# DrSleep/nas-segm-pytorch

Hardware: AMD Instinct MI355X
Metric: images/sec (fwd+bwd+optimizer step) WACV arch0 2048x1024 bs=4/GPU (higher is better)
Workload: dtype f32

## Files before the change

### nas-segm-pytorch_amd/csrc/irdw.hip

```cpp
#include "dw_common.h"

namespace {

#ifndef NASSEG_IR_BWD_MINB
#define NASSEG_IR_BWD_MINB 1
#endif
#ifndef NASSEG_IR_FWD_MINB
#define NASSEG_IR_FWD_MINB 1
#endif
constexpr int kIrMaxTiles = 12;
constexpr int kIrMaxWaves = 4;

__device__ __forceinline__ f32x4 mfma16(float a, float b, f32x4 c) {
  return __builtin_amdgcn_mfma_f32_16x16x4f32(a, b, c, 0, 0, 0);
}

template <int CTRL>
__device__ __forceinline__ float dpp_shift0(float v) {
  return __int_as_float(__builtin_amdgcn_update_dpp(0, __float_as_int(v), CTRL, 0xF, 0xF, true));
}
__device__ __forceinline__ float4 from_left(float4 v) {
  return make_float4(dpp_shift0<0x111>(v.x), dpp_shift0<0x111>(v.y), dpp_shift0<0x111>(v.z), dpp_shift0<0x111>(v.w));
}
__device__ __forceinline__ float4 from_right(float4 v) {
  return make_float4(dpp_shift0<0x101>(v.x), dpp_shift0<0x101>(v.y), dpp_shift0<0x101>(v.z), dpp_shift0<0x101>(v.w));
}
__device__ __forceinline__ float4 round_like_storage(float4 v) {
#ifdef NASSEG_BF16
  v = make_float4(bf16_to_f32(f32_to_bf16(v.x)), bf16_to_f32(f32_to_bf16(v.y)), bf16_to_f32(f32_to_bf16(v.z)),
                  bf16_to_f32(f32_to_bf16(v.w)));
#endif
  return v;
}

struct IrCommon {
  const act_t* x;
  const float* w1;
  const float* in_scale;
  const float* in_shift;
  int in_act;
  const float* sc1;
  const float* sh1;
  int act1;
  int B, H, W, K, C, Ho, Wo;
  int strips, chunks, rows_per_chunk, items;
};

template <int KT, bool PRO>
struct IrLane {
  float aw[KT][4];
  int koff[KT];
  float4 psc[KT], psh[KT];
  float plo, phi;
};
template <int KT, bool PRO>
__device__ __forceinline__ IrLane<KT, PRO> ir_lane(const IrCommon& q, int t, int j, int kg) {
  IrLane<KT, PRO> l;
#pragma unroll
  for (int kb = 0; kb < KT; ++kb) {
    const int k0 = 16 * kb + 4 * kg;
    const bool kok = k0 < q.K;
    l.koff[kb] = kok ? k0 : 0;
#pragma unroll
    for (int c = 0; c < 4; ++c) l.aw[kb][c] = kok ? q.w1[(size_t)(16 * t + j) * q.K + k0 + c] : 0.f;
    if (PRO) {
      l.psc[kb] = (q.in_scale && kok) ? ld4(q.in_scale + k0) : make_float4(1.f, 1.f, 1.f, 1.f);
      l.psh[kb] = (q.in_shift && kok) ? ld4(q.in_shift + k0) : f4zero();
    }
  }
  l.plo = q.in_act ? 0.f : -INFINITY;
  l.phi = q.in_act == NASSEG_ACT_RELU6 ? 6.f : INFINITY;
  return l;
}
template <int KT, bool PRO>
struct IrRawX {
  float4 v[KT];
};
template <int KT, bool PRO>
__device__ __forceinline__ IrRawX<KT, PRO> ir_load(const IrLane<KT, PRO>& l, const act_t* xp) {
  IrRawX<KT, PRO> r;
#pragma unroll
  for (int kb = 0; kb < KT; ++kb) r.v[kb] = lda4(xp + l.koff[kb]);
  return r;
}
template <int KT, bool PRO>
__device__ __forceinline__ float4 ir_mma(const IrLane<KT, PRO>& l, const IrRawX<KT, PRO>& r) {
  f32x4 acc = (f32x4){0.f, 0.f, 0.f, 0.f};
#pragma unroll
  for (int kb = 0; kb < KT; ++kb) {
    float4 v = r.v[kb];
    if (PRO) {
      v = fma4(v, l.psc[kb], l.psh[kb]);
      v.x = __builtin_amdgcn_fmed3f(v.x, l.plo, l.phi);
      v.y = __builtin_amdgcn_fmed3f(v.y, l.plo, l.phi);
      v.z = __builtin_amdgcn_fmed3f(v.z, l.plo, l.phi);
      v.w = __builtin_amdgcn_fmed3f(v.w, l.plo, l.phi);
    }
    acc = mfma16(l.aw[kb][0], v.x, acc);
    acc = mfma16(l.aw[kb][1], v.y, acc);
    acc = mfma16(l.aw[kb][2], v.z, acc);
    acc = mfma16(l.aw[kb][3], v.w, acc);
  }
  return round_like_storage(make_float4(acc[0], acc[1], acc[2], acc[3]));
}

struct IrFwdArgs {
  IrCommon c;
  const float* wdw;
  act_t* z2;
  float* stats;
};

template <int STRIDE, int KT, bool PRO>
__global__ __launch_bounds__(64 * kIrMaxWaves, NASSEG_IR_FWD_MINB) void irdw_fwd_kernel(IrFwdArgs a) {
  const IrCommon& q = a.c;
  const int lane = threadIdx.x & 63, t = blockIdx.y * (blockDim.x >> 6) + (threadIdx.x >> 6);
  const int j = lane & 15, kg = lane >> 4;
  const int C = q.C, K = q.K, H = q.H, W = q.W, Ho = q.Ho, Wo = q.Wo;
  const int c4 = 4 * t + kg;
  const IrLane<KT, PRO> ln = ir_lane<KT, PRO>(q, t, j, kg);
  const float4 sc1 = ld4(q.sc1 + 4 * c4), sh1 = ld4(q.sh1 + 4 * c4);
  const float lo1 = q.act1 ? 0.f : -INFINITY, hi1 = q.act1 == NASSEG_ACT_RELU6 ? 6.f : INFINITY;
  float4 wd[9];
#pragma unroll
  for (int tp = 0; tp < 9; ++tp) wd[tp] = ld4(a.wdw + (size_t)tp * C + 4 * c4);
  double dsum[4] = {0.0, 0.0, 0.0, 0.0}, dsq[4] = {0.0, 0.0, 0.0, 0.0};
  const bool out_lane = STRIDE == 1 ? (j >= 1 && j <= 14) : ((j & 1) && j <= 13);

  for (int item = blockIdx.x; item < q.items; item += gridDim.x) {
    const int s = item % q.strips;
    const int rest = item / q.strips;
    const int ch = rest % q.chunks, b = rest / q.chunks;
    const int oy0 = ch * q.rows_per_chunk;
    const int oy1 = oy0 + q.rows_per_chunk < Ho ? oy0 + q.rows_per_chunk : Ho;
    const int col = 14 * s - 1 + j;
    const bool colok = col >= 0 && col < W;
    const int colc = col < 0 ? 0 : (col >= W ? W - 1 : col);
    const int ox = STRIDE == 1 ? col : 7 * s + (j >> 1);
    const bool outok = out_lane && ox < Wo;
    const act_t* xb = q.x + ((size_t)b * H * W + colc) * K;
    act_t* zb = a.z2 + ((size_t)b * Ho * Wo + (outok ? ox : 0)) * C + 4 * c4;
    float4 fs = f4zero(), fq = f4zero();
    auto fetch = [&](int iy) {
      return ir_load<KT, PRO>(ln, xb + (size_t)(iy < 0 ? 0 : (iy >= H ? H - 1 : iy)) * W * K);
    };
    auto make_row = [&](const IrRawX<KT, PRO>& raw, int iy, float4& L, float4& M, float4& R) {
      const float4 z = ir_mma<KT, PRO>(ln, raw);
      float4 a1 = fma4(z, sc1, sh1);
      a1.x = __builtin_amdgcn_fmed3f(a1.x, lo1, hi1);
      a1.y = __builtin_amdgcn_fmed3f(a1.y, lo1, hi1);
      a1.z = __builtin_amdgcn_fmed3f(a1.z, lo1, hi1);
      a1.w = __builtin_amdgcn_fmed3f(a1.w, lo1, hi1);
      a1 = keep_if(a1, colok && iy >= 0 && iy < H);
      M = a1;
      L = from_left(a1);
      R = from_right(a1);
    };
    auto emit = [&](int oy, const float4& A0, const float4& A1, const float4& A2, const float4& B0, const float4& B1,
                    const float4& B2, const float4& C0, const float4& C1, const float4& C2) {
      float4 o = mul4(wd[0], A0);
      o = fma4(wd[1], A1, o);
      o = fma4(wd[2], A2, o);
      o = fma4(wd[3], B0, o);
      o = fma4(wd[4], B1, o);
      o = fma4(wd[5], B2, o);
      o = fma4(wd[6], C0, o);
      o = fma4(wd[7], C1, o);
      o = fma4(wd[8], C2, o);
      if (outok) sta4(zb + (size_t)oy * Wo * C, o);
      const float4 m = keep_if(o, outok);
      fs = add4(fs, m);
      fq = fma4(m, m, fq);
    };
    float4 L0, M0, R0, L1, M1, R1, L2, M2, R2;
    if (STRIDE == 1) {
      IrRawX<KT, PRO> ra = fetch(oy0 - 1), rb = fetch(oy0);
      make_row(ra, oy0 - 1, L0, M0, R0);
      ra = fetch(oy0 + 1);
      make_row(rb, oy0, L1, M1, R1);
      int oy = oy0;
      for (; oy + 2 < oy1; oy += 3) {
        rb = fetch(oy + 2);
        make_row(ra, oy + 1, L2, M2, R2);
        emit(oy, L0, M0, R0, L1, M1, R1, L2, M2, R2);
        ra = fetch(oy + 3);
        make_row(rb, oy + 2, L0, M0, R0);
        emit(oy + 1, L1, M1, R1, L2, M2, R2, L0, M0, R0);
        rb = fetch(oy + 4);
        make_row(ra, oy + 3, L1, M1, R1);
        emit(oy + 2, L2, M2, R2, L0, M0, R0, L1, M1, R1);
        ra = rb;
      }
      if (oy < oy1) {
        rb = fetch(oy + 2);
        make_row(ra, oy + 1, L2, M2, R2);
        emit(oy, L0, M0, R0, L1, M1, R1, L2, M2, R2);
        if (oy + 1 < oy1) {
          make_row(rb, oy + 2, L0, M0, R0);
          emit(oy + 1, L1, M1, R1, L2, M2, R2, L0, M0, R0);
        }
      }
    } else {
      IrRawX<KT, PRO> ra = fetch(2 * oy0 - 1), rb = fetch(2 * oy0);
      make_row(ra, 2 * oy0 - 1, L0, M0, R0);
      ra = fetch(2 * oy0 + 1);
      int oy = oy0;
      for (; oy + 1 < oy1; oy += 2) {
        make_row(rb, 2 * oy, L1, M1, R1);
        rb = fetch(2 * oy + 2);
        make_row(ra, 2 * oy + 1, L2, M2, R2);
        ra = fetch(2 * oy + 3);
        emit(oy, L0, M0, R0, L1, M1, R1, L2, M2, R2);
        make_row(rb, 2 * oy + 2, L1, M1, R1);
        rb = fetch(2 * oy + 4);
        make_row(ra, 2 * oy + 3, L0, M0, R0);
        ra = fetch(2 * oy + 5);
        emit(oy + 1, L2, M2, R2, L1, M1, R1, L0, M0, R0);
      }
      if (oy < oy1) {
        make_row(rb, 2 * oy, L1, M1, R1);
        make_row(ra, 2 * oy + 1, L2, M2, R2);
        emit(oy, L0, M0, R0, L1, M1, R1, L2, M2, R2);
      }
    }
    dsum[0] += (double)fs.x; dsum[1] += (double)fs.y; dsum[2] += (double)fs.z; dsum[3] += (double)fs.w;
    dsq[0] += (double)fq.x; dsq[1] += (double)fq.y; dsq[2] += (double)fq.z; dsq[3] += (double)fq.w;
  }
#pragma unroll
  for (int r = 0; r < 4; ++r) {
    dsum[r] = row16_allsum(dsum[r]);
    dsq[r] = row16_allsum(dsq[r]);
  }
  if (j == 0) {
    float* row = a.stats + (size_t)blockIdx.x * 2 * C + 4 * c4;
    *reinterpret_cast<float4*>(row) = make_float4((float)dsum[0], (float)dsum[1], (float)dsum[2], (float)dsum[3]);
    *reinterpret_cast<float4*>(row + C) = make_float4((float)dsq[0], (float)dsq[1], (float)dsq[2], (float)dsq[3]);
  }
}

struct IrBwdArgs {
  IrCommon c;
  const float* mu1;
  const float* is1;
  const act_t* g;
  const act_t* z2;
  const float* wdw;
  int flip;
  act_t* ge;
  float* partial;
  float* stats;
  const float* sc2; const float* sh2; const float* mu2; const float* is2; const float* sums2;
  int train2, act2;
  float invM;
};

struct IrDz {
  float4 ca, cb, cd, cs;
};
__device__ __forceinline__ IrDz ir_dz_const(const IrBwdArgs& a, int c4) {
  IrDz k;
  const int C = a.c.C;
  k.ca = ld4(a.sc2 + c4 * 4);
  k.cs = a.act2 ? ld4(a.sh2 + c4 * 4) : f4zero();
  k.cb = f4zero();
  k.cd = f4zero();
  if (a.train2) {
    const float4 is = ld4(a.is2 + c4 * 4), mu = ld4(a.mu2 + c4 * 4);
    const float4 s0 = ld4(a.sums2 + c4 * 4), s1 = ld4(a.sums2 + C + c4 * 4);
    const float m = a.invM;
    k.cb = make_float4(-k.ca.x * is.x * (s1.x * m), -k.ca.y * is.y * (s1.y * m), -k.ca.z * is.z * (s1.z * m),
                       -k.ca.w * is.w * (s1.w * m));
    k.cd = make_float4(k.ca.x * (mu.x * is.x * (s1.x * m) - s0.x * m), k.ca.y * (mu.y * is.y * (s1.y * m) - s0.y * m),
                       k.ca.z * (mu.z * is.z * (s1.z * m) - s0.z * m), k.ca.w * (mu.w * is.w * (s1.w * m) - s0.w * m));
  }
  return k;
}
struct IrRaw {
  float4 g, z;
  bool ok;
};
__device__ __forceinline__ IrRaw ir_dz_load(const IrBwdArgs& a, int b, int oy, int ox, int c4) {
  IrRaw r;
  const int Ho = a.c.Ho, Wo = a.c.Wo;
  r.ok = oy >= 0 && oy < Ho && ox >= 0 && ox < Wo;
  const int oyc = oy < 0 ? 0 : (oy >= Ho ? Ho - 1 : oy), oxc = ox < 0 ? 0 : (ox >= Wo ? Wo - 1 : ox);
  const size_t off = (((size_t)b * Ho + oyc) * Wo + oxc) * a.c.C + c4 * 4;
  r.g = lda4(a.g + off);
  r.z = lda4(a.z2 + off);
  return r;
}
__device__ __forceinline__ float4 ir_dz_make(const ActSel& act2, const IrDz& k, const IrRaw& r) {
  const float4 y = fma4(r.z, k.ca, k.cs);
  const float4 gv = make_float4(r.g.x * act_mask(y.x, act2), r.g.y * act_mask(y.y, act2), r.g.z * act_mask(y.z, act2),
                                r.g.w * act_mask(y.w, act2));
  return keep_if(round_like_storage(fma4(gv, k.ca, fma4(r.z, k.cb, k.cd))), r.ok);
}

template <int STRIDE, int KT, bool PRO>
__global__ __launch_bounds__(64 * kIrMaxWaves, NASSEG_IR_BWD_MINB) void irdw_bwd_kernel(IrBwdArgs a) {
  const IrCommon& q = a.c;
  const int lane = threadIdx.x & 63, t = blockIdx.y * (blockDim.x >> 6) + (threadIdx.x >> 6);
  const int j = lane & 15, kg = lane >> 4;
  const int C = q.C, K = q.K, H = q.H, W = q.W;
  const int c4 = 4 * t + kg;
  const IrLane<KT, PRO> ln = ir_lane<KT, PRO>(q, t, j, kg);
  const float4 sc1 = ld4(q.sc1 + 4 * c4), sh1 = ld4(q.sh1 + 4 * c4);
  const float4 mu1 = ld4(a.mu1 + 4 * c4), is1 = ld4(a.is1 + 4 * c4);
  const float lo1 = q.act1 ? 0.f : -INFINITY, hi1 = q.act1 == NASSEG_ACT_RELU6 ? 6.f : INFINITY;
  const IrDz kc = ir_dz_const(a, c4);
  const ActSel sel1 = act_sel(q.act1), sel2 = act_sel(a.act2);
  float4 lw[9];
#pragma unroll
  for (int tp = 0; tp < 9; ++tp) lw[tp] = ld4(a.wdw + (size_t)(a.flip ? 8 - tp : tp) * C + 4 * c4);
  float4 dwa[9];
#pragma unroll
  for (int tp = 0; tp < 9; ++tp) dwa[tp] = f4zero();
  float4 ssum[2] = {f4zero(), f4zero()};
  auto finish = [&](float4& o, float4 z1, bool ok) {
    const float4 y = fma4(z1, sc1, sh1);
    o.x *= act_mask(y.x, sel1);
    o.y *= act_mask(y.y, sel1);
    o.z *= act_mask(y.z, sel1);
    o.w *= act_mask(y.w, sel1);
    const float4 v = keep_if(o, ok);
    const float4 xh = make_float4((z1.x - mu1.x) * is1.x, (z1.y - mu1.y) * is1.y, (z1.z - mu1.z) * is1.z,
                                  (z1.w - mu1.w) * is1.w);
    ssum[0] = add4(ssum[0], v);
    ssum[1] = fma4(v, xh, ssum[1]);
  };
  auto activated = [&](float4 z1) {
    float4 v = fma4(z1, sc1, sh1);
    v.x = __builtin_amdgcn_fmed3f(v.x, lo1, hi1);
    v.y = __builtin_amdgcn_fmed3f(v.y, lo1, hi1);
    v.z = __builtin_amdgcn_fmed3f(v.z, lo1, hi1);
    v.w = __builtin_amdgcn_fmed3f(v.w, lo1, hi1);
    return v;
  };

  for (int item = blockIdx.x; item < q.items; item += gridDim.x) {
    const int s = item % q.strips;
    const int rest = item / q.strips;
    const int ch = rest % q.chunks, b = rest / q.chunks;
    const int r0 = ch * q.rows_per_chunk;
    if (STRIDE == 1) {
      const int r1 = r0 + q.rows_per_chunk < H ? r0 + q.rows_per_chunk : H;
      const int ix = 14 * s - 1 + j;
      const bool live = j >= 1 && j <= 14 && ix < W;
      const int xc = ix < 0 ? 0 : (ix >= W ? W - 1 : ix);
      const bool colok = ix >= 0 && ix < W;
      const act_t* xcol = q.x + ((size_t)b * H * W + xc) * K;
      float4 dl[3], dm[3], dr[3];
      auto make_dz = [&](const IrRaw& raw, float4& L, float4& M, float4& R) {
        IrRaw r = raw;
        r.ok = r.ok && colok;
        M = ir_dz_make(sel2, kc, r);
        L = from_left(M);
        R = from_right(M);
      };
      make_dz(ir_dz_load(a, b, r0 - 1, xc, c4), dl[1], dm[1], dr[1]);
      make_dz(ir_dz_load(a, b, r0, xc, c4), dl[2], dm[2], dr[2]);
      IrRaw nxt = ir_dz_load(a, b, r0 + 1, xc, c4), nxt2 = ir_dz_load(a, b, r0 + 2, xc, c4);
      IrRawX<KT, PRO> xnxt = ir_load<KT, PRO>(ln, xcol + (size_t)r0 * W * K);
      IrRawX<KT, PRO> xnxt2 = ir_load<KT, PRO>(ln, xcol + (size_t)(r0 + 1 < H ? r0 + 1 : H - 1) * W * K);
      for (int iy = r0; iy < r1; ++iy) {
        const IrRaw cur = nxt;
        const IrRawX<KT, PRO> xcur = xnxt;
        nxt = nxt2;
        xnxt = xnxt2;
        nxt2 = ir_dz_load(a, b, iy + 3, xc, c4);
        xnxt2 = ir_load<KT, PRO>(ln, xcol + (size_t)(iy + 2 < H ? iy + 2 : H - 1) * W * K);
        const float4 z1 = ir_mma<KT, PRO>(ln, xcur);
        dl[0] = dl[1]; dm[0] = dm[1]; dr[0] = dr[1];
        dl[1] = dl[2]; dm[1] = dm[2]; dr[1] = dr[2];
        make_dz(cur, dl[2], dm[2], dr[2]);
        const float4 xa = keep_if(activated(z1), live);
        float4 o = f4zero();
#pragma unroll
        for (int ty = 0; ty < 3; ++ty) {
          o = fma4(lw[ty * 3 + 0], dr[2 - ty], o);
          dwa[ty * 3 + 0] = fma4(xa, dr[2 - ty], dwa[ty * 3 + 0]);
          o = fma4(lw[ty * 3 + 1], dm[2 - ty], o);
          dwa[ty * 3 + 1] = fma4(xa, dm[2 - ty], dwa[ty * 3 + 1]);
          o = fma4(lw[ty * 3 + 2], dl[2 - ty], o);
          dwa[ty * 3 + 2] = fma4(xa, dl[2 - ty], dwa[ty * 3 + 2]);
        }
        finish(o, z1, live);
        if (live) sta4(a.ge + (((size_t)b * H + iy) * W + ix) * C + c4 * 4, o);
      }
    } else {
      const int Hq = (H + 1) >> 1, Wq = (W + 1) >> 1;
      const int r1 = r0 + q.rows_per_chunk < Hq ? r0 + q.rows_per_chunk : Hq;
      const int xq = 15 * s + j;
      const bool live = j <= 14 && xq < Wq;
      const int xqc = xq < Wq ? xq : Wq - 1;
      float4 d[2][2];
      auto make_dz = [&](const IrRaw& raw, float4& M, float4& R) {
        M = ir_dz_make(sel2, kc, raw);
        R = from_right(M);
      };
      auto fetch_quad = [&](int aq, IrRawX<KT, PRO> (&dst)[2][2]) {
#pragma unroll
        for (int py = 0; py < 2; ++py)
#pragma unroll
          for (int px = 0; px < 2; ++px) {
            const int iy = 2 * aq + py, ix = 2 * xqc + px;
            dst[py][px] = ir_load<KT, PRO>(ln, q.x + (((size_t)b * H + (iy < H ? iy : H - 1)) * W + (ix < W ? ix : W - 1)) * K);
          }
      };
      make_dz(ir_dz_load(a, b, r0, xq, c4), d[1][0], d[1][1]);
      IrRaw nxt = ir_dz_load(a, b, r0 + 1, xq, c4);
      IrRawX<KT, PRO> xnxt[2][2];
      fetch_quad(r0, xnxt);
      for (int aq = r0; aq < r1; ++aq) {
        const IrRaw cur = nxt;
        IrRawX<KT, PRO> xcur[2][2];
#pragma unroll
        for (int py = 0; py < 2; ++py)
#pragma unroll
          for (int px = 0; px < 2; ++px) xcur[py][px] = xnxt[py][px];
        nxt = ir_dz_load(a, b, aq + 2, xq, c4);
        fetch_quad(aq + 1 < Hq ? aq + 1 : aq, xnxt);
        d[0][0] = d[1][0];
        d[0][1] = d[1][1];
        make_dz(cur, d[1][0], d[1][1]);
#pragma unroll
        for (int py = 0; py < 2; ++py)
#pragma unroll
          for (int px = 0; px < 2; ++px) {
            const int iy = 2 * aq + py, ix = 2 * xqc + px;
            const bool ok = live && iy < H && ix < W;
            const float4 z1 = ir_mma<KT, PRO>(ln, xcur[py][px]);
            const float4 xa = keep_if(activated(z1), ok);
            float4 o = f4zero();
#pragma unroll
            for (int ty = 0; ty < 3; ++ty)
#pragma unroll
              for (int tx = 0; tx < 3; ++tx) {
                if (((ty + 1) & 1) != py || ((tx + 1) & 1) != px) continue;
                const int ry = (py + 1 - ty) / 2, rx = (px + 1 - tx) / 2;
                const float4 dv = d[ry][rx];
                o = fma4(lw[ty * 3 + tx], dv, o);
                dwa[ty * 3 + tx] = fma4(xa, dv, dwa[ty * 3 + tx]);
              }
            finish(o, z1, ok);
            if (ok) sta4(a.ge + (((size_t)b * H + iy) * W + 2 * xq + px) * C + c4 * 4, o);
          }
      }
    }
  }
#pragma unroll
  for (int tp = 0; tp < 9; ++tp) {
    float4 v = dwa[tp];
    v = make_float4(row16_allsum(v.x), row16_allsum(v.y), row16_allsum(v.z), row16_allsum(v.w));
    if (j == 0) *reinterpret_cast<float4*>(a.partial + ((size_t)blockIdx.x * 9 + tp) * C + 4 * c4) = v;
  }
#pragma unroll
  for (int r = 0; r < 2; ++r) {
    float4 v = ssum[r];
    v = make_float4(row16_allsum(v.x), row16_allsum(v.y), row16_allsum(v.z), row16_allsum(v.w));
    if (j == 0) *reinterpret_cast<float4*>(a.stats + ((size_t)blockIdx.x * 2 + r) * C + 4 * c4) = v;
  }
}


constexpr int kMomTile = 64;
constexpr int kMomGrid = 512;
constexpr int kMomSamples = 16;

template <int KT, bool PRO>
__global__ __launch_bounds__(256) void ir_moments_kernel(const act_t* __restrict__ x, const float* __restrict__ in_scale,
                                                         const float* __restrict__ in_shift, int in_act, int K, int M,
                                                         float* __restrict__ rows, float* __restrict__ pivot) {
  constexpr int KP = 16 * KT, Q = KP / 4, LSK = KP + 4, IT = (kMomTile * Q) / 256;
  __shared__ float xs[kMomTile * LSK];
  __shared__ float red[KP * KP > 256 * 4 ? KP * KP : 256 * 4];
  __shared__ float pvs[KP];
  const int tid = threadIdx.x, lane = tid & 63, wave = tid >> 6;
  const int j = lane & 15, kg = lane >> 4;
  const int quad = tid % Q, k0 = 4 * quad;
  const bool kok = k0 < K;
  float4 psc = make_float4(1.f, 1.f, 1.f, 1.f), psh = f4zero();
  if (PRO && kok) {
    if (in_scale) psc = ld4(in_scale + k0);
    if (in_shift) psh = ld4(in_shift + k0);
  }
  const float plo = in_act ? 0.f : -INFINITY, phi = in_act == NASSEG_ACT_RELU6 ? 6.f : INFINITY;
  auto prologue = [&](float4 v) {
    if (PRO) {
      v = fma4(v, psc, psh);
      v.x = __builtin_amdgcn_fmed3f(v.x, plo, phi);
      v.y = __builtin_amdgcn_fmed3f(v.y, plo, phi);
      v.z = __builtin_amdgcn_fmed3f(v.z, plo, phi);
      v.w = __builtin_amdgcn_fmed3f(v.w, plo, phi);
    }
    return v;
  };
  f32x4 acc[KT][KT];
#pragma unroll
  for (int ta = 0; ta < KT; ++ta)
#pragma unroll
    for (int tb = 0; tb < KT; ++tb) acc[ta][tb] = (f32x4){0.f, 0.f, 0.f, 0.f};
  float4 csum = f4zero();
  const int ntiles = (M + kMomTile - 1) / kMomTile;
  float4 raw[IT];
  auto issue = [&](int tile) {
#pragma unroll
    for (int u = 0; u < IT; ++u) {
      const int p = tile * kMomTile + (tid + 256 * u) / Q;
      raw[u] = lda4(x + (size_t)(p < M ? p : M - 1) * K + (kok ? k0 : 0));
    }
  };
  if ((int)blockIdx.x < ntiles) issue(blockIdx.x);
  float4 piv = f4zero();
  if (wave == 0) {
    if (kok) {
      float4 smp[kMomSamples];
#pragma unroll
      for (int i = 0; i < kMomSamples; ++i)
        smp[i] = lda4(x + (size_t)(((int64_t)i * M) / kMomSamples) * K + k0);
      piv = prologue(smp[0]);
      float4 dev = f4zero();
#pragma unroll
      for (int i = 1; i < kMomSamples; ++i) {
        const float4 v = prologue(smp[i]);
        dev.x = fmaxf(dev.x, fabsf(v.x - piv.x));
        dev.y = fmaxf(dev.y, fabsf(v.y - piv.y));
        dev.z = fmaxf(dev.z, fabsf(v.z - piv.z));
        dev.w = fmaxf(dev.w, fabsf(v.w - piv.w));
      }
      piv.x = fabsf(piv.x) > dev.x ? piv.x : 0.f;
      piv.y = fabsf(piv.y) > dev.y ? piv.y : 0.f;
      piv.z = fabsf(piv.z) > dev.z ? piv.z : 0.f;
      piv.w = fabsf(piv.w) > dev.w ? piv.w : 0.f;
    }
    if (lane < Q) *reinterpret_cast<float4*>(&pvs[k0]) = piv;
  }
  __syncthreads();
  piv = *reinterpret_cast<const float4*>(&pvs[k0]);
  for (int tile = blockIdx.x; tile < ntiles; tile += gridDim.x) {
#pragma unroll
    for (int u = 0; u < IT; ++u) {
      const int px = (tid + 256 * u) / Q;
      float4 v = prologue(raw[u]);
      v = make_float4(v.x - piv.x, v.y - piv.y, v.z - piv.z, v.w - piv.w);
      v = keep_if(v, kok && tile * kMomTile + px < M);
      *reinterpret_cast<float4*>(&xs[px * LSK + k0]) = v;
      csum = add4(csum, v);
    }
    __syncthreads();
    if (tile + (int)gridDim.x < ntiles) issue(tile + gridDim.x);
#pragma unroll
    for (int q4 = 0; q4 < 4; ++q4) {
      const float* row = &xs[(4 * (4 * wave + q4) + kg) * LSK + j];
      float a[KT];
#pragma unroll
      for (int ta = 0; ta < KT; ++ta) a[ta] = row[16 * ta];
#pragma unroll
      for (int ta = 0; ta < KT; ++ta)
#pragma unroll
        for (int tb = 0; tb < KT; ++tb) acc[ta][tb] = mfma16(a[ta], a[tb], acc[ta][tb]);
    }
    __syncthreads();
  }
  float* out = rows + (size_t)blockIdx.x * (KP * KP + KP);
  for (int w = 0; w < 4; ++w) {
    if (wave == w) {
#pragma unroll
      for (int ta = 0; ta < KT; ++ta)
#pragma unroll
        for (int tb = 0; tb < KT; ++tb)
#pragma unroll
          for (int i = 0; i < 4; ++i) {
            float* slot = &red[(16 * ta + 4 * kg + i) * KP + 16 * tb + j];
            *slot = (w == 0 ? 0.f : *slot) + acc[ta][tb][i];
          }
    }
    __syncthreads();
  }
  for (int e = tid; e < KP * KP; e += 256) out[e] = red[e];
  __syncthreads();
  *reinterpret_cast<float4*>(&red[4 * tid]) = csum;
  __syncthreads();
  if (tid < KP) {
    const int qd = tid >> 2, c = tid & 3;
    float sacc = 0.f;
    for (int u = qd; u < 256; u += Q) sacc += red[4 * u + c];
    out[KP * KP + tid] = sacc;
  }
  if (blockIdx.x == 0 && tid < Q) *reinterpret_cast<float4*>(pivot + k0) = piv;
}

__global__ __launch_bounds__(256) void ir_moments_finalize(const float* __restrict__ mom, const float* __restrict__ pivot,
                                                           const float* __restrict__ w1,
                                                           int K, int KP, int C, double M, float eps, float momentum,
                                                           const float* __restrict__ gamma, const float* __restrict__ beta,
                                                           float* __restrict__ mean, float* __restrict__ invstd,
                                                           float* __restrict__ scale, float* __restrict__ shift,
                                                           float* __restrict__ running_mean,
                                                           float* __restrict__ running_var, int64_t* nbt) {
  __shared__ float S[32 * 32 + 32];
  __shared__ float cv[32];
  __shared__ float wn[8][32];
  for (int e = threadIdx.x; e < KP * KP + KP; e += 256) S[e] = mom[e];
  if (threadIdx.x < 32) cv[threadIdx.x] = (int)threadIdx.x < KP ? pivot[threadIdx.x] : 0.f;
  const int nl = threadIdx.x >> 5, k = threadIdx.x & 31;
  const int n = blockIdx.x * 8 + nl;
  wn[nl][k] = (n < C && k < K) ? w1[(size_t)n * K + k] : 0.f;
  __syncthreads();
  if (blockIdx.x == 0 && threadIdx.x == 0 && nbt) *nbt += 1;
  const double wk = (double)wn[nl][k];
  double r = 0.0;
  if (k < K) {
    for (int l = 0; l < K; ++l) r += (double)S[k * KP + l] * (double)wn[nl][l];
  }
  double wsw = wk * r, ws = k < K ? wk * (double)S[KP * KP + k] : 0.0, wc = k < K ? wk * (double)cv[k] : 0.0;
#pragma unroll
  for (int off = 16; off >= 1; off >>= 1) {
    wsw += __shfl_xor(wsw, off);
    ws += __shfl_xor(ws, off);
    wc += __shfl_xor(wc, off);
  }
  if (n >= C || k != 0) return;
  const double dmu = ws / M;
  const double mu = wc + dmu;
  double var = wsw / M - dmu * dmu;
  if (var < 0.0) var = 0.0;
  const double is = 1.0 / sqrt(var + (double)eps);
  mean[n] = (float)mu;
  invstd[n] = (float)is;
  const double g = gamma ? (double)gamma[n] : 1.0;
  const double bt = beta ? (double)beta[n] : 0.0;
  scale[n] = (float)(g * is);
  shift[n] = (float)(bt - mu * g * is);
  if (running_mean) {
    running_mean[n] = (float)((1.0 - momentum) * (double)running_mean[n] + momentum * mu);
    const double unb = M > 1.0 ? var * M / (M - 1.0) : var;
    running_var[n] = (float)((1.0 - momentum) * (double)running_var[n] + momentum * unb);
  }
}

struct IrPlan {
  int ok, kt, waves, groups, strips, chunks, rows_per_chunk, items, grid;
};
inline IrPlan ir_plan(int B, int H, int W, int K, int C, int stride, bool backward) {
  IrPlan p = {};
  if (B <= 0 || H <= 0 || W <= 0 || K % 4 || K < 4 || K > 32 || C % 16 || C < 16 || C > 16 * kIrMaxTiles ||
      (stride != 1 && stride != 2))
    return p;
  const int Ho = (H - 1) / stride + 1, Wo = (W - 1) / stride + 1;
  p.kt = K <= 16 ? 1 : 2;
  const int tiles = C / 16;
  p.waves = tiles % 4 == 0 ? 4 : (tiles % 3 == 0 ? 3 : (tiles % 2 == 0 ? 2 : 1));
  p.groups = tiles / p.waves;
  int rows;
  if (!backward) {
    p.strips = stride == 1 ? cdiv(W, 14) : cdiv(Wo, 7);
    rows = Ho;
  } else {
    p.strips = stride == 1 ? cdiv(W, 14) : cdiv((W + 1) / 2, 15);
    rows = stride == 1 ? H : (H + 1) / 2;
  }
  const int resident = 256 * 2;
  int rpc = 64;
  while (rpc > 8 && (int64_t)B * cdiv(rows, rpc) * p.strips < 4LL * resident) rpc >>= 1;
  p.rows_per_chunk = rpc;
  p.chunks = cdiv(rows, rpc);
  const int64_t items = (int64_t)B * p.chunks * p.strips;
  if (items >= 2147483647LL) return p;
  p.items = (int)items;
  p.grid = p.items < resident ? p.items : resident;
  p.ok = 1;
  return p;
}

}

extern "C" {

#if NASSEG_FP32_ONLY
int64_t nasseg_irdw_rows(int B, int H, int W, int K, int C, int stride, int backward) {
  const IrPlan p = ir_plan(B, H, W, K, C, stride, backward != 0);
  return p.ok ? p.grid : 0;
}
int64_t nasseg_irdw_config(int B, int H, int W, int K, int C, int stride, int backward) {
  const IrPlan p = ir_plan(B, H, W, K, C, stride, backward != 0);
  return p.ok ? 1000 * p.waves + 10 * p.groups + p.kt : 0;
}
#endif

#if NASSEG_FP32_ONLY
int64_t nasseg_irdw_stats_workspace(int K) {
  const int KP = K <= 16 ? 16 : 32;
  return (int64_t)(kMomGrid + 64 + 1) * (KP * KP + KP) + KP;
}
#endif

int NASSEG_FN(irdw_stats)(const act_t* x, const float* w1, const float* in_scale, const float* in_shift, int in_act,
                          int B, int H, int W, int K, int C, float eps, float momentum, const float* gamma,
                          const float* beta, float* mean, float* invstd, float* scale, float* shift,
                          float* running_mean, float* running_var, int64_t* num_batches_tracked, float* ws,
                          void* stream) {
  NASSEG_REQUIRE(x && w1 && mean && invstd && scale && shift && ws, "irdw_stats: null tensor");
  NASSEG_REQUIRE(B > 0 && H > 0 && W > 0 && K >= 4 && K <= 32 && K % 4 == 0 && C > 0, "irdw_stats: bad shape");
  const int64_t M64 = (int64_t)B * H * W;
  NASSEG_REQUIRE(M64 < 2147483647LL, "irdw_stats: too many pixels");
  const int M = (int)M64;
  const int KP = K <= 16 ? 16 : 32, per = KP * KP + KP;
  const int ntiles = (M + kMomTile - 1) / kMomTile;
  const int grid = ntiles < kMomGrid ? ntiles : kMomGrid;
  const bool pro = in_scale || in_shift || in_act;
  hipStream_t s = (hipStream_t)stream;
  float* total = ws + (size_t)(kMomGrid + 64) * per;
  float* pivot = total + per;
  if (KP == 16 && pro) hipLaunchKernelGGL((ir_moments_kernel<1, true>), dim3(grid), dim3(256), 0, s, x, in_scale, in_shift, in_act, K, M, ws, pivot);
  else if (KP == 16) hipLaunchKernelGGL((ir_moments_kernel<1, false>), dim3(grid), dim3(256), 0, s, x, in_scale, in_shift, in_act, K, M, ws, pivot);
  else if (pro) hipLaunchKernelGGL((ir_moments_kernel<2, true>), dim3(grid), dim3(256), 0, s, x, in_scale, in_shift, in_act, K, M, ws, pivot);
  else hipLaunchKernelGGL((ir_moments_kernel<2, false>), dim3(grid), dim3(256), 0, s, x, in_scale, in_shift, in_act, K, M, ws, pivot);
  NASSEG_LAUNCH_CHECK("ir_moments_kernel");
  const int rc = nasseg_rows_sum(ws, grid, per, total, stream);
  if (rc != NASSEG_OK) return rc;
  hipLaunchKernelGGL(ir_moments_finalize, dim3(cdiv(C, 8)), dim3(256), 0, s, total, pivot, w1, K, KP, C, (double)M, eps, momentum,
                     gamma, beta, mean, invstd, scale, shift, running_mean, running_var, num_batches_tracked);
  NASSEG_LAUNCH_CHECK("ir_moments_finalize");
  return NASSEG_OK;
}

#define IR_LAUNCH(KERNEL, ARGS)                                                                              \
  do {                                                                                                       \
    const dim3 grid(p.grid, p.groups), block(64 * p.waves);                                                            \
    if (stride == 1 && p.kt == 1 && pro) hipLaunchKernelGGL((KERNEL<1, 1, true>), grid, block, 0, s, ARGS);  \
    else if (stride == 1 && p.kt == 1) hipLaunchKernelGGL((KERNEL<1, 1, false>), grid, block, 0, s, ARGS);   \
    else if (stride == 1 && pro) hipLaunchKernelGGL((KERNEL<1, 2, true>), grid, block, 0, s, ARGS);          \
    else if (stride == 1) hipLaunchKernelGGL((KERNEL<1, 2, false>), grid, block, 0, s, ARGS);                \
    else if (p.kt == 1 && pro) hipLaunchKernelGGL((KERNEL<2, 1, true>), grid, block, 0, s, ARGS);            \
    else if (p.kt == 1) hipLaunchKernelGGL((KERNEL<2, 1, false>), grid, block, 0, s, ARGS);                  \
    else if (pro) hipLaunchKernelGGL((KERNEL<2, 2, true>), grid, block, 0, s, ARGS);                         \
    else hipLaunchKernelGGL((KERNEL<2, 2, false>), grid, block, 0, s, ARGS);                                 \
  } while (0)

static void ir_fill_common(IrCommon& c, const act_t* x, const float* w1, const float* in_scale, const float* in_shift,
                           int in_act, const float* sc1, const float* sh1, int act1, int B, int H, int W, int K, int C,
                           int Ho, int Wo, const IrPlan& p) {
  c.x = x; c.w1 = w1; c.in_scale = in_scale; c.in_shift = in_shift; c.in_act = in_act;
  c.sc1 = sc1; c.sh1 = sh1; c.act1 = act1;
  c.B = B; c.H = H; c.W = W; c.K = K; c.C = C; c.Ho = Ho; c.Wo = Wo;
  c.strips = p.strips; c.chunks = p.chunks; c.rows_per_chunk = p.rows_per_chunk; c.items = p.items;
}

int NASSEG_FN(irdw_fwd)(const act_t* x, const float* w1, const float* wdw, act_t* z2, const float* in_scale,
                        const float* in_shift, int in_act, const float* bn1_scale, const float* bn1_shift, int act1,
                        int B, int H, int W, int K, int C, int Ho, int Wo, int stride, float* stats, void* stream) {
  NASSEG_REQUIRE(x && w1 && wdw && z2 && bn1_scale && bn1_shift && stats, "irdw_fwd: null tensor");
  const IrPlan p = ir_plan(B, H, W, K, C, stride, false);
  NASSEG_REQUIRE(p.ok, "irdw_fwd: geometry not served (K=%d C=%d stride %d)", K, C, stride);
  NASSEG_REQUIRE(Ho == (H - 1) / stride + 1 && Wo == (W - 1) / stride + 1, "irdw_fwd: output size does not match");
  IrFwdArgs a = {};
  ir_fill_common(a.c, x, w1, in_scale, in_shift, in_act, bn1_scale, bn1_shift, act1, B, H, W, K, C, Ho, Wo, p);
  a.wdw = wdw; a.z2 = z2; a.stats = stats;
  const bool pro = in_scale || in_shift || in_act;
  hipStream_t s = (hipStream_t)stream;
  IR_LAUNCH(irdw_fwd_kernel, a);
  NASSEG_LAUNCH_CHECK("irdw_fwd_kernel");
  return NASSEG_OK;
}

int NASSEG_FN(irdw_bwd)(const act_t* x, const float* w1, const act_t* g, const act_t* z2, const float* wdw,
                        int wdw_flipped, act_t* ge, float* dw, float* ws, const float* in_scale,
                        const float* in_shift, int in_act, const float* bn1_scale, const float* bn1_shift,
                        const float* bn1_mean, const float* bn1_invstd, int act1, const float* bn2_scale,
                        const float* bn2_shift, const float* bn2_mean, const float* bn2_invstd,
                        const float* bn2_sums, int bn2_train, int bn2_act, int B, int H, int W, int K, int C, int Ho,
                        int Wo, int stride, float* stats, void* stream) {
  NASSEG_REQUIRE(x && w1 && g && z2 && wdw && ge && ws && stats && bn1_scale && bn1_shift && bn1_mean && bn1_invstd &&
                     bn2_scale,
                 "irdw_bwd: null tensor");
  NASSEG_REQUIRE((!bn2_train || (bn2_mean && bn2_invstd && bn2_sums)) && (!bn2_act || bn2_shift),
                 "irdw_bwd: missing BatchNorm tensors");
  const IrPlan p = ir_plan(B, H, W, K, C, stride, true);
  NASSEG_REQUIRE(p.ok, "irdw_bwd: geometry not served (K=%d C=%d stride %d)", K, C, stride);
  NASSEG_REQUIRE(Ho == (H - 1) / stride + 1 && Wo == (W - 1) / stride + 1, "irdw_bwd: output size does not match");
  IrBwdArgs a = {};
  ir_fill_common(a.c, x, w1, in_scale, in_shift, in_act, bn1_scale, bn1_shift, act1, B, H, W, K, C, Ho, Wo, p);
  a.mu1 = bn1_mean; a.is1 = bn1_invstd; a.g = g; a.z2 = z2; a.wdw = wdw; a.flip = wdw_flipped != 0;
  a.ge = ge; a.partial = ws; a.stats = stats;
  a.sc2 = bn2_scale; a.sh2 = bn2_shift; a.mu2 = bn2_mean; a.is2 = bn2_invstd; a.sums2 = bn2_sums;
  a.train2 = bn2_train; a.act2 = bn2_act;
  a.invM = (float)(1.0 / ((double)B * Ho * Wo));
  const bool pro = in_scale || in_shift || in_act;
  hipStream_t s = (hipStream_t)stream;
  IR_LAUNCH(irdw_bwd_kernel, a);
  NASSEG_LAUNCH_CHECK("irdw_bwd_kernel");
  if (!dw) return NASSEG_OK;
  const float* parts[1] = {ws};
  float* outs[1] = {dw};
  const int dims[5] = {p.grid, 9, C, 1, 0};
  return nasseg_wgrad_finalize_many(1, parts, outs, dims, stream);
}

}
```

Before: 307.9.

## Share stride-2 input loads across waves via LDS double-buffered ring in IR-dw backward

In the stride-2 backward path, the per-wave quad fetch of the expand input is replaced by a cooperative scheme. Each wave loads a share of the input pixel units, applies the prologue affine+clamp once, and writes them into a double-buffered shared-memory ring that every wave reads back. Batches are separated by block barriers. The intent is to spread global load latency across waves and avoid repeating prologue math, at the cost of LDS traffic, extra __syncthreads and added LDS footprint that may lower occupancy.

```diff
diff --git a/nas-segm-pytorch_amd/csrc/irdw.hip b/nas-segm-pytorch_amd/csrc/irdw.hip
--- a/nas-segm-pytorch_amd/csrc/irdw.hip
+++ b/nas-segm-pytorch_amd/csrc/irdw.hip
@@ -84,18 +84,26 @@
   return r;
 }
 template <int KT, bool PRO>
-__device__ __forceinline__ float4 ir_mma(const IrLane<KT, PRO>& l, const IrRawX<KT, PRO>& r) {
-  f32x4 acc = (f32x4){0.f, 0.f, 0.f, 0.f};
-#pragma unroll
-  for (int kb = 0; kb < KT; ++kb) {
-    float4 v = r.v[kb];
-    if (PRO) {
-      v = fma4(v, l.psc[kb], l.psh[kb]);
+__device__ __forceinline__ IrRawX<KT, PRO> ir_prep(const IrLane<KT, PRO>& l, IrRawX<KT, PRO> r) {
+  if (PRO) {
+#pragma unroll
+    for (int kb = 0; kb < KT; ++kb) {
+      float4 v = fma4(r.v[kb], l.psc[kb], l.psh[kb]);
       v.x = __builtin_amdgcn_fmed3f(v.x, l.plo, l.phi);
       v.y = __builtin_amdgcn_fmed3f(v.y, l.plo, l.phi);
       v.z = __builtin_amdgcn_fmed3f(v.z, l.plo, l.phi);
       v.w = __builtin_amdgcn_fmed3f(v.w, l.plo, l.phi);
-    }
+      r.v[kb] = v;
+    }
+  }
+  return r;
+}
+template <int KT, bool PRO>
+__device__ __forceinline__ float4 ir_mma_prepared(const IrLane<KT, PRO>& l, const IrRawX<KT, PRO>& r) {
+  f32x4 acc = (f32x4){0.f, 0.f, 0.f, 0.f};
+#pragma unroll
+  for (int kb = 0; kb < KT; ++kb) {
+    const float4 v = r.v[kb];
     acc = mfma16(l.aw[kb][0], v.x, acc);
     acc = mfma16(l.aw[kb][1], v.y, acc);
     acc = mfma16(l.aw[kb][2], v.z, acc);
@@ -103,6 +111,64 @@
   }
   return round_like_storage(make_float4(acc[0], acc[1], acc[2], acc[3]));
 }
+template <int KT, bool PRO>
+__device__ __forceinline__ float4 ir_mma(const IrLane<KT, PRO>& l, const IrRawX<KT, PRO>& r) {
+  return ir_mma_prepared<KT, PRO>(l, ir_prep<KT, PRO>(l, r));
+}
+
+template <int KT, bool PRO, int UPW, class Addr>
+struct IrRows {
+  const IrLane<KT, PRO>& ln;
+  float4* ring;
+  const Addr& addr;
+  int nw, wave, total;
+  IrRawX<KT, PRO> g[UPW];
+  int nb, left, rd;
+  __device__ __forceinline__ void request(int batch, IrRawX<KT, PRO> (&dst)[UPW]) {
+#pragma unroll
+    for (int i = 0; i < UPW; ++i) {
+      const int u = (batch * UPW + i) * nw + wave;
+      if (u < total) dst[i] = ir_load<KT, PRO>(ln, addr(u));
+    }
+  }
+  __device__ __forceinline__ void put(int batch, const IrRawX<KT, PRO> (&src)[UPW]) {
+#pragma unroll
+    for (int i = 0; i < UPW; ++i) {
+      if ((batch * UPW + i) * nw + wave < total) {
+        const IrRawX<KT, PRO> r = ir_prep<KT, PRO>(ln, src[i]);
+#pragma unroll
+        for (int kb = 0; kb < KT; ++kb) ring[((((batch & 1) * UPW + i) * nw + wave) * KT + kb) * 64] = r.v[kb];
+      }
+    }
+  }
+  __device__ __forceinline__ void start(int units) {
+    total = units;
+    IrRawX<KT, PRO> g0[UPW];
+    request(0, g0);
+    request(1, g);
+    __syncthreads();
+    put(0, g0);
+    nb = 0;
+    left = 0;
+    rd = 0;
+  }
+  __device__ __forceinline__ IrRawX<KT, PRO> next() {
+    if (left == 0) {
+      __syncthreads();
+      put(nb + 1, g);
+      request(nb + 2, g);
+      rd = (nb & 1) * UPW * nw * KT * 64;
+      left = UPW * nw;
+      ++nb;
+    }
+    IrRawX<KT, PRO> r;
+#pragma unroll
+    for (int kb = 0; kb < KT; ++kb) r.v[kb] = ring[rd + kb * 64];
+    rd += KT * 64;
+    --left;
+    return r;
+  }
+};
 
 struct IrFwdArgs {
   IrCommon c;
@@ -299,7 +365,10 @@
 template <int STRIDE, int KT, bool PRO>
 __global__ __launch_bounds__(64 * kIrMaxWaves, NASSEG_IR_BWD_MINB) void irdw_bwd_kernel(IrBwdArgs a) {
   const IrCommon& q = a.c;
-  const int lane = threadIdx.x & 63, t = blockIdx.y * (blockDim.x >> 6) + (threadIdx.x >> 6);
+  constexpr int UPW = KT == 1 ? 4 : 2;
+  __shared__ float4 ring_s[STRIDE == 2 ? 2 * UPW * kIrMaxWaves * KT * 64 : 1];
+  const int lane = threadIdx.x & 63, nw = blockDim.x >> 6, wave = __builtin_amdgcn_readfirstlane(threadIdx.x >> 6);
+  const int t = blockIdx.y * nw + wave;
   const int j = lane & 15, kg = lane >> 4;
   const int C = q.C, K = q.K, H = q.H, W = q.W;
   const int c4 = 4 * t + kg;
@@ -398,28 +467,22 @@
         M = ir_dz_make(sel2, kc, raw);
         R = from_right(M);
       };
-      auto fetch_quad = [&](int aq, IrRawX<KT, PRO> (&dst)[2][2]) {
-#pragma unroll
-        for (int py = 0; py < 2; ++py)
-#pragma unroll
-          for (int px = 0; px < 2; ++px) {
-            const int iy = 2 * aq + py, ix = 2 * xqc + px;
-            dst[py][px] = ir_load<KT, PRO>(ln, q.x + (((size_t)b * H + (iy < H ? iy : H - 1)) * W + (ix < W ? ix : W - 1)) * K);
-          }
+      auto addr = [&](int u) {
+        const int iy = 2 * (r0 + (u >> 2)) + ((u >> 1) & 1), ix = 2 * xqc + (u & 1);
+        return q.x + (((size_t)b * H + (iy < H ? iy : H - 1)) * W + (ix < W ? ix : W - 1)) * K;
       };
+      IrRows<KT, PRO, UPW, decltype(addr)> rows = {ln, ring_s + lane, addr, nw, wave};
+      rows.start(4 * (r1 - r0));
       make_dz(ir_dz_load(a, b, r0, xq, c4), d[1][0], d[1][1]);
       IrRaw nxt = ir_dz_load(a, b, r0 + 1, xq, c4);
-      IrRawX<KT, PRO> xnxt[2][2];
-      fetch_quad(r0, xnxt);
       for (int aq = r0; aq < r1; ++aq) {
         const IrRaw cur = nxt;
+        nxt = ir_dz_load(a, b, aq + 2, xq, c4);
         IrRawX<KT, PRO> xcur[2][2];
 #pragma unroll
         for (int py = 0; py < 2; ++py)
 #pragma unroll
-          for (int px = 0; px < 2; ++px) xcur[py][px] = xnxt[py][px];
-        nxt = ir_dz_load(a, b, aq + 2, xq, c4);
-        fetch_quad(aq + 1 < Hq ? aq + 1 : aq, xnxt);
+          for (int px = 0; px < 2; ++px) xcur[py][px] = rows.next();
         d[0][0] = d[1][0];
         d[0][1] = d[1][1];
         make_dz(cur, d[1][0], d[1][1]);
@@ -429,7 +492,7 @@
           for (int px = 0; px < 2; ++px) {
             const int iy = 2 * aq + py, ix = 2 * xqc + px;
             const bool ok = live && iy < H && ix < W;
-            const float4 z1 = ir_mma<KT, PRO>(ln, xcur[py][px]);
+            const float4 z1 = ir_mma_prepared<KT, PRO>(ln, xcur[py][px]);
             const float4 xa = keep_if(activated(z1), ok);
             float4 o = f4zero();
 #pragma unroll
```

After: 307.0. Within noise of the previous version (-0.3%).
